# zgbkdlm/fbs

Hardware: AMD Instinct MI355X
Metric: particle-steps/sec (N x T per Gibbs sweep) (higher is better)
Workload: dtype f32; 1 GPU; 2-D Gaussian bridge toy (BASELINE config 2): N=65536 particles, T=500 steps, ts=linspace(0,2), analytic score, gibbs_kernel eb=True ef=False marg_y=False, conditional killing resampling; one step = one Gibbs sweep of a batch of 4 chain(s) (reference driver default nchains=4, vmapped); nparticles=65536, nsteps=500, nchains=4, du=1, dv=1, parallelism=1 GPU(s) x 4 independent chain(s) each, no collective

## Files before the change

### fbs_amd/csrc/fbsmi_lg.hip

```cpp
#include <hip/hip_runtime.h>

#include <array>
#include <cmath>
#include <cstdlib>
#include <map>
#include <mutex>
#include <new>
#include <string>
#include <utility>
#include <vector>

#include "../../include/fbsmi.h"
#include "fbsmi_device.h"
#include "fbsmi_em_path.h"
#include "fbsmi_host.h"

namespace fbsmi {

constexpr int kMaxNbSweep = 1024;
constexpr int kNumProfKernels = 3;

struct LgDev {
    int C;
    int Ctot, c0;
// ... 1183 lines not shown
        }
        __syncthreads();
        t2[0] = waves_combine(L.xch[0][0], L.xch[0][1], L.xch[0][2], L.xch[0][3], s2[0], p2[0]);
        t2[1] = waves_combine(L.xch[1][0], L.xch[1][1], L.xch[1][2], L.xch[1][3], s2[1], p2[1]);
    }
    rootW = t2[0];
    last = d.plus1 ? t2[0] + e.xw : t2[0];
    const float Ji = fmaxf(1.0f - (d.plus1 ? t2[1] + e.xj : t2[1]), 0.0f);
    if (tid) L.topW[g] = make_float2(tree_left_sum(p2[0], tid), e.wf);
    const float tile_ref = tree_fold(Ji, e.refsib);
    float bsib[8];
    {
        const int wb = b_ref >> 6;
#pragma unroll
        for (int lv = 0; lv < 6; ++lv) bsib[lv] = L.bc[lv];
        bsib[6] = L.xch[1][wb ^ 1];
        bsib[7] = (wb & 2) ? L.xch[1][0] + L.xch[1][1] : L.xch[1][2] + L.xch[1][3];
    }
    const float rootJ = ref_extra ? t2[1] : tree_fold(tile_ref, bsib);
    const float lastJ = d.plus1 ? rootJ + (ref_extra ? Ji : e.xj) : rootJ;
    if (tid) {
        const int c = __builtin_ctz(tid);
        const bool hit = !ref_extra && b_ref < tid && b_ref >= tid - (1 << c);
        const float left = hit ? tree_fold(tile_ref, bsib, c) : tree_left_sum(p2[1], tid);
        const float jw = d.plus1 ? jprob_at(e.wf, w_max, d.N) : jprob_pow2(e.wf, w_max, inv_n);
        const float jf = tid * kBlock == i_ref ? Ji : (tid < nb ? jw : 0.0f);
        L.topJ[g] = make_float2(left, jf);
    }
    __syncthreads();
    const float q = lastJ * (1.0f - u3);
    const int top_levels = 31 - __builtin_clz(nb);
    float P = 0.0f, E = rootJ;
    int h = tree_walk_n(L.topJ, kBlock / nb, top_levels, q, P, E);
    const int lo0 = (h - kBlock) * kBlock;
    const float wj = d.w[lo0 + tid];
    float s1[1], t1s[1];
    TreePath p1[1];
    s1[0] = lo0 + tid == i_ref ? Ji : (d.plus1 ? jprob_at(wj, w_max, d.N) : jprob_pow2(wj, w_max, inv_n));
    const float xj = s1[0];
    block_upsweep_n<1>(s1, p1, L.xch[4], t1s);
    if (tid) L.tileJ[g] = make_float2(tree_left_sum(p1[0], tid), xj);
    __syncthreads();
    h = tree_walk_n(L.tileJ, 1, 6, q, P, E);
    {
        const float2 a = L.tileJ[h];
        const float4 c = *reinterpret_cast<const float4*>(L.tileJ + 2 * h);
        const bool g1 = tree_walk(a, q, P, E);
        const float tt = P + (g1 ? c.x : c.z);
        const bool gl = q <= E;
        E = gl ? tt : E;
        h = 4 * h + (g1 ? 0 : 2) + (gl ? 0 : 1);
    }
    const int leaf = lo0 + h - kBlock;
    return q <= E ? leaf : leaf + 1;
}

__device__ __forceinline__ void tree_search_lds(const TreeLds& L, int nb, float q, float& P, float& E, int& tile, int& h) {
    h = tree_walk_n(L.topW, kBlock / nb, 31 - __builtin_clz(nb), q, P, E);
    tile = h - kBlock;
    h = tree_walk_n(L.midW + tile * kMidN, 1, kMidLv, q, P, E);
}

struct TreeRound {
    float s1, y1, s2l, y2l, s2r, y2r, s3a, y3a, s3b, y3b, s3c, y3c, s3d, y3d;
};

__device__ __forceinline__ TreeRound tree_round_load(const LgDev& d, int tile, int h) {
    const float2* tr = d.trW + (size_t)tile * kTreeNodes;
    const float2 n1 = tr[h];
    const float4 n2 = *reinterpret_cast<const float4*>(tr + 2 * h);
    if constexpr (kMidLv == 4) {
        return TreeRound{n1.x, n1.y, n2.x, n2.y, n2.z, n2.w, 0.f, 0.f, 0.f, 0.f, 0.f, 0.f, 0.f, 0.f};
    } else {
        const float4 n3a = *reinterpret_cast<const float4*>(tr + 4 * h);
        const float4 n3b = *reinterpret_cast<const float4*>(tr + 4 * h + 2);
        return TreeRound{n1.x, n1.y, n2.x, n2.y, n2.z, n2.w, n3a.x, n3a.y, n3a.z, n3a.w, n3b.x, n3b.y, n3b.z, n3b.w};
    }
}

__device__ __forceinline__ int tree_round_walk(const TreeRound r, int tile, int h, float q, float& P, float& E) {
    static_assert(kMidLv == 3 || kMidLv == 4, "the round covers the levels between the LDS part and the last four leaves");
    const bool g1 = tree_walk(make_float2(r.s1, r.y1), q, P, E);
    const bool g2 = tree_walk(make_float2(g1 ? r.s2l : r.s2r, g1 ? r.y2l : r.y2r), q, P, E);
    int h4 = 4 * h + (g1 ? 0 : 2) + (g2 ? 0 : 1);
    if constexpr (kMidLv == 3) {
        const float s3 = g1 ? (g2 ? r.s3a : r.s3b) : (g2 ? r.s3c : r.s3d);
        const float y3 = g1 ? (g2 ? r.y3a : r.y3b) : (g2 ? r.y3c : r.y3d);
        h4 = 2 * h4 + (tree_walk(make_float2(s3, y3), q, P, E) ? 0 : 1);
    }
    return tile * kBlock + (h4 - 64) * 4;
}

__device__ __forceinline__ int tree_leaves_walk(float4 w4, int lo, float q, float P, float E) {
    const bool g4 = tree_walk(make_float2(w4.x + w4.y, w4.z), q, P, E);
    const float tt = P + (g4 ? w4.x : w4.z);
    const bool g5 = q <= E;
    const float e1 = g5 ? tt : E;
    const int leaf = lo + (g4 ? 0 : 2) + (g5 ? 0 : 1);
    return q <= e1 ? leaf : leaf + 1;
}

template <int DMAX>
constexpr bool kEarlyRow = DMAX <= 2;

template <int DMAX>
__device__ __forceinline__ int tree_redraw(const LgDev& d, const float* up, int tile, int h, float q, float P, float E,
                                           float (&ucand)[DMAX]) {
    const int N = d.N;
    const TreeRound rd = tree_round_load(d, tile, h);
    const int lo = tree_round_walk(rd, tile, h, q, P, E);
    const float4 w4 = *reinterpret_cast<const float4*>(d.w + lo);
    float4 ug[DMAX];
    float ue[DMAX];
    if (kEarlyRow<DMAX>) {
        const int en = lo + 4 < N ? lo + 4 : N - 1;
#pragma unroll
        for (int r = 0; r < DMAX; ++r) {
            ug[r] = r < d.du ? *reinterpret_cast<const float4*>(up + (size_t)r * N + lo) : make_float4(0.f, 0.f, 0.f, 0.f);
            ue[r] = r < d.du ? up[(size_t)r * N + en] : 0.0f;
        }
    }
    const int red = tree_leaves_walk(w4, lo, q, P, E);
    if (kEarlyRow<DMAX>) {
        const int k = red - lo;
#pragma unroll
        for (int r = 0; r < DMAX; ++r) {
            const float lo2 = (k & 1) ? ug[r].y : ug[r].x, hi2 = (k & 1) ? ug[r].w : ug[r].z;
            ucand[r] = k >= 4 ? ue[r] : ((k & 2) ? hi2 : lo2);
        }
    }
    return red;
}

__device__ __forceinline__ int tree_build_shared(const LgDev& d, const TreeEntry& e, TreeLds& L, bool builder, int i_ref, float u3,
                                                 float w_max, float inv_n, float& last) {
    __shared__ int Jsh;
    __shared__ float lastsh;
    if (builder) {
        float lastb, rootW;
        const int J = tree_build(d, e, L, i_ref, u3, w_max, inv_n, lastb, rootW);
        if (threadIdx.x == 0) {
            Jsh = J;
            lastsh = lastb;
        }
    } else {
#pragma unroll
        for (int k = 0; k < kTreeBuildBarriers; ++k) __syncthreads();
    }
    __syncthreads();
    last = lastsh;
    return Jsh;
}

template <int DMAX, int HALVES>
__global__ void __launch_bounds__(kBlock * HALVES) k_lg_prop1t(LgDev dd, int s) {
    const LgDev d = chain_view(dd, blockIdx.y);
    __shared__ TreeLds L;
    __shared__ float part[2][4 * HALVES];
    const int N = d.N, tid = threadIdx.x & (kBlock - 1), half = threadIdx.x / kBlock;
    int bx = blockIdx.x;
    if (dd.pin) {
        if (blockIdx.x & 7) return;
        bx = blockIdx.x >> 3;
    }
    const int tileb = bx * HALVES + half;
    const int m = tileb * kBlock + tid;
    const bool live = m < N;
    GibbsStep<DMAX> g = gibbs_step_entry<DMAX>(d, s);
    const float w_max = d.scal[1];
    const float inv_n = 1.0f / (float)N;
    TreeEntry te{};
    if (half == 0) te = tree_entry_loads(d);
    gibbs_step_entry_rows<DMAX>(d, s, g);
    float xi[DMAX];
#pragma unroll
    for (int r = 0; r < DMAX; ++r)
        xi[r] = r < d.du ? normal_at(g.t0, g.t1, (uint64_t)N * d.du, (uint64_t)(live ? m : 0) * d.du + r) : 0.0f;
    float last, rootW;
    int J;
    if (HALVES == 1) {
        J = tree_build(d, te, L, g.i_ref, g.u3, w_max, inv_n, last, rootW);
    } else {
        J = tree_build_shared(d, te, L, half == 0, g.i_ref, g.u3, w_max, inv_n, last);
        rootW = last;
    }
    const int src = live ? roll_source(m, roll_shift(g.j_ref, J, N), N) : 0;
    const float ws = d.w[src];
    float u[DMAX];
    load_row<DMAX>(d, g.up, src, u);
    const float u1 = uniform_at(g.a0, g.a1, (uint64_t)N, (uint64_t)src);
    const float u2 = uniform_at(g.b0, g.b1, (uint64_t)N, (uint64_t)src);
    const float q = last * (1.0f - u2);
    float P = 0.0f, E = rootW;
    int tile, h, red = 0;
    tree_search_lds(L, d.nb - d.plus1, q, P, E, tile, h);
    const bool killed = live && u1 * w_max >= ws;
    float ucand[DMAX];
    if (killed) red = tree_redraw<DMAX>(d, g.up, tile, h, q, P, E, ucand);
    gibbs_slot_gather<DMAX, kEarlyRow<DMAX>>(d, g, s, m, src, killed, red, u, ucand, live);
    const float l = gibbs_slot_finish<DMAX>(d, g, s, m, u, xi, live);
    float mx, sx;
    block_lse_partial_tiles(l, part[0], part[1], mx, sx);
    if (tid == 0) {
        d.bmax[tileb] = mx;
        d.bsumexp[tileb] = sx;
    }
}

template <int DMAX>
constexpr bool kPairNoise = DMAX <= 4;

template <int DMAX, int HALVES>
__global__ void __launch_bounds__(kBlock * HALVES) k_lg_prop1tp(LgDev dd, int s) {
    static_assert(HALVES == 2 || HALVES == 4, "two sides of HALVES / 2 tiles");
    constexpr int HP = HALVES / 2, NP = kBlock * HP;
    const LgDev d = chain_view(dd, blockIdx.y);
    __shared__ TreeLds L;
    __shared__ float part[2][4 * HALVES];
    __shared__ float xish[kPairNoise<DMAX> ? DMAX : 1][NP];
    const int N = d.N, tid = threadIdx.x & (kBlock - 1), half = threadIdx.x / kBlock;
    const bool upper = half >= HP;
    const int pr = (int)threadIdx.x - (upper ? NP : 0);
    const int mL = blockIdx.x * NP + pr;
    const int m = upper ? mL + (N >> 1) : mL;
    const int tileb = m / kBlock;
    GibbsStep<DMAX> g = gibbs_step_entry<DMAX>(d, s);
    const float w_max = d.scal[1];
    const float inv_n = 1.0f / (float)N;
    TreeEntry te{};
    if (half == 0) te = tree_entry_loads(d);
    gibbs_step_entry_rows<DMAX>(d, s, g);
    float xi[DMAX] = {};
    if (!kPairNoise<DMAX>) {
#pragma unroll
        for (int r = 0; r < DMAX; ++r)
            if (r < d.du) xi[r] = normal_at(g.t0, g.t1, (uint64_t)N * d.du, (uint64_t)m * d.du + r);
    } else if (upper) {
#pragma unroll
        for (int r = 0; r < DMAX; ++r) {
            if (r < d.du) {
                uint32_t lo_, hi_;
                random_bits_pair(g.t0, g.t1, (uint64_t)N * d.du, (uint64_t)mL * d.du + r, lo_, hi_);
                xish[r][pr] = normal_from_bits(lo_);
                xi[r] = normal_from_bits(hi_);
            }
        }
    }
    float last;
    const int J = tree_build_shared(d, te, L, half == 0, g.i_ref, g.u3, w_max, inv_n, last);
    const int src = roll_source(m, roll_shift(g.j_ref, J, N), N);
    const float ws = d.w[src];
    float u[DMAX];
    load_row<DMAX>(d, g.up, src, u);
    if (kPairNoise<DMAX> && !upper) {
#pragma unroll
        for (int r = 0; r < DMAX; ++r)
            if (r < d.du) xi[r] = xish[r][pr];
    }
    const float u1 = uniform_at(g.a0, g.a1, (uint64_t)N, (uint64_t)src);
    const float u2 = uniform_at(g.b0, g.b1, (uint64_t)N, (uint64_t)src);
    const float q = last * (1.0f - u2);
    float P = 0.0f, E = last;
    int tile, h, red = 0;
    tree_search_lds(L, d.nb, q, P, E, tile, h);
    const bool killed = u1 * w_max >= ws;
    float ucand[DMAX];
    if (killed) red = tree_redraw<DMAX>(d, g.up, tile, h, q, P, E, ucand);
    gibbs_slot_gather<DMAX, kEarlyRow<DMAX>>(d, g, s, m, src, killed, red, u, ucand);
    const float l = gibbs_slot_finish<DMAX>(d, g, s, m, u, xi);
    float mx, sx;
    block_lse_partial_tiles(l, part[0], part[1], mx, sx);
    if (tid == 0) {
        d.bmax[tileb] = mx;
        d.bsumexp[tileb] = sx;
    }
}

__device__ __forceinline__ float halfwave_max(float m) {
    m = fmaxf(m, tree_partner<1>(m));
    m = fmaxf(m, tree_partner<2>(m));
    m = fmaxf(m, tree_partner<4>(m));
    m = fmaxf(m, tree_partner<8>(m));
    m = fmaxf(m, tree_partner<16>(m));
    return m;
}

__device__ __forceinline__ float halfwave_sum(float s) {
    const int lane = threadIdx.x & 63;
#define FBSMI_HALFWAVE_LEVEL(m, M)                      \
    {                                                   \
        const float o_ = tree_partner<M>(s);            \
        s = ((lane >> m) & 1) ? o_ + s : s + o_;        \
    }
    FBSMI_HALFWAVE_LEVEL(0, 1)
    FBSMI_HALFWAVE_LEVEL(1, 2)
    FBSMI_HALFWAVE_LEVEL(2, 4)
    FBSMI_HALFWAVE_LEVEL(3, 8)
    FBSMI_HALFWAVE_LEVEL(4, 16)
#undef FBSMI_HALFWAVE_LEVEL
    return s;
}

template <int DMAX, int HALVES>
__global__ void __launch_bounds__(kBlock * HALVES) k_lg_prop1th(LgDev dd, int s) {
    static_assert(HALVES == 2 || HALVES == 4, "two sides of HALVES / 2 tiles");
    constexpr int HP = HALVES / 2, NP = kBlock * HP;
    const LgDev d = chain_view(dd, blockIdx.y);
    __shared__ TreeLds L;
    __shared__ __attribute__((aligned(16))) float part[2][2][HP][8];
    __shared__ float xish[kPairNoise<DMAX> ? DMAX : 1][2 * NP];
    const int N = d.N, hN = N >> 1, tid = threadIdx.x, lane = threadIdx.x & 63, wv = threadIdx.x >> 6;
    const int hw = lane >> 5;
    const bool builder = tid < kBlock;
    const int pr = wv * 32 + (lane & 31);
    const int mL = blockIdx.x * NP + pr;
    const int m = mL + (hw ? hN : 0);
    const int ts = wv >> 3, bk = wv & 7;
    const int tileb = blockIdx.x * HP + ts + (hw ? d.nb >> 1 : 0);
    GibbsStep<DMAX> g = gibbs_step_entry<DMAX>(d, s);
    const float w_max = d.scal[1];
    const float inv_n = 1.0f / (float)N;
    TreeEntry te{};
    if (builder) te = tree_entry_loads(d);
    gibbs_step_entry_rows<DMAX>(d, s, g);
    float xi[DMAX] = {};
    if (!kPairNoise<DMAX>) {
#pragma unroll
        for (int r = 0; r < DMAX; ++r)
            if (r < d.du) xi[r] = normal_at(g.t0, g.t1, (uint64_t)N * d.du, (uint64_t)m * d.du + r);
    } else if (tid >= NP) {
        const int p = tid - NP, own = (p >> 5) * 64 + (p & 31);
        const int mp = blockIdx.x * NP + p;
#pragma unroll
        for (int r = 0; r < DMAX; ++r) {
            if (r < d.du) {
                uint32_t lo_, hi_;
                random_bits_pair(g.t0, g.t1, (uint64_t)N * d.du, (uint64_t)mp * d.du + r, lo_, hi_);
                xish[r][own] = normal_from_bits(lo_);
                xish[r][own + 32] = normal_from_bits(hi_);
            }
        }
    }
    float last;
    const int J = tree_build_shared(d, te, L, builder, g.i_ref, g.u3, w_max, inv_n, last);
    const int src = roll_source(m, roll_shift(g.j_ref, J, N), N);
    const float ws = d.w[src];
    float u[DMAX];
    load_row<DMAX>(d, g.up, src, u);
    if (kPairNoise<DMAX>) {
#pragma unroll
        for (int r = 0; r < DMAX; ++r)
            if (r < d.du) xi[r] = xish[r][tid];
    }
    const int c = src & (hN - 1);
    const bool swp = (src >= hN) != (hw != 0);
    uint32_t o0, o1;
    threefry2x32(hw ? g.b0 : g.a0, hw ? g.b1 : g.a1, (uint32_t)c, (uint32_t)(c + hN), o0, o1);
    const auto xw = __builtin_amdgcn_permlane32_swap(swp ? o1 : o0, swp ? o0 : o1, false, false);
    const float u1 = fbsmi_bits_to_unit(xw[0]);
    const float u2 = fbsmi_bits_to_unit(xw[1]);
    const float q = last * (1.0f - u2);
    float P = 0.0f, E = last;
    int tile, h, red = 0;
    tree_search_lds(L, d.nb, q, P, E, tile, h);
    const bool killed = u1 * w_max >= ws;
    float ucand[DMAX];
    if (killed) red = tree_redraw<DMAX>(d, g.up, tile, h, q, P, E, ucand);
    gibbs_slot_gather<DMAX, kEarlyRow<DMAX>>(d, g, s, m, src, killed, red, u, ucand);
    const float l = gibbs_slot_finish<DMAX>(d, g, s, m, u, xi);
    float mx, sx;
    {
        const float mw = halfwave_max(l);
        if ((lane & 31) == 0) part[0][hw][ts][bk] = mw;
        __syncthreads();
        const float4 ma = *reinterpret_cast<const float4*>(&part[0][hw][ts][0]);
        const float4 mb = *reinterpret_cast<const float4*>(&part[0][hw][ts][4]);
        mx = fmaxf(fmaxf(fmaxf(ma.x, ma.y), fmaxf(ma.z, ma.w)), fmaxf(fmaxf(mb.x, mb.y), fmaxf(mb.z, mb.w)));
        const float sw_ = halfwave_sum(fbsmi_expf(l - finite_or_zero_f(mx)));
        if ((lane & 31) == 0) part[1][hw][ts][bk] = sw_;
        __syncthreads();
        const float4 sa = *reinterpret_cast<const float4*>(&part[1][hw][ts][0]);
        const float4 sb = *reinterpret_cast<const float4*>(&part[1][hw][ts][4]);
        sx = ((sa.x + sa.y) + (sa.z + sa.w)) + ((sb.x + sb.y) + (sb.z + sb.w));
    }
    if (bk == 0 && (lane & 31) == 0) {
        d.bmax[tileb] = mx;
        d.bsumexp[tileb] = sx;
    }
}

template <int DMAX>
__global__ void __launch_bounds__(kBlock) k_lg_prop2t(LgDev dd, int s) {
    const LgDev d = chain_view(dd, blockIdx.y);
    __shared__ TreeLds L;
    __shared__ float xch2[2][8];
    const int N = d.N, tid = threadIdx.x;
    const int mA = blockIdx.x * kBlock + tid;
    const int m[2] = {mA, mA + (N >> 1)};
    GibbsStep<DMAX> g = gibbs_step_entry<DMAX>(d, s);
    const float w_max = d.scal[1];
    const float inv_n = 1.0f / (float)N;
    const TreeEntry te = tree_entry_loads(d);
    gibbs_step_entry_rows<DMAX>(d, s, g);
    float xi[2][DMAX];
    pair_noise<DMAX>(d, g, mA, xi[0], xi[1]);
    float last;
    float rootW_unused;
    const int J = tree_build(d, te, L, g.i_ref, g.u3, w_max, inv_n, last, rootW_unused);
    int src[2];
    pair_sources(mA, g.j_ref, J, N, src);
    float ws[2], u[2][DMAX];
#pragma unroll
    for (int h2 = 0; h2 < 2; ++h2) {
        ws[h2] = d.w[src[h2]];
#pragma unroll
        for (int r = 0; r < DMAX; ++r) u[h2][r] = r < d.du ? g.up[(size_t)r * N + src[h2]] : 0.0f;
    }
    float u1[2], u2[2];
    pair_uniforms<DMAX>(g, N, src, u1, u2);
    const float qK[2] = {last * (1.0f - u2[0]), last * (1.0f - u2[1])};
    float P[2] = {0.0f, 0.0f}, E[2] = {last, last};
    int tile[2], h[2], hi[2] = {0, 0};
    {
        auto walk2x2 = [&](const float2* hp0, const float2* hp1, int& h0, int& h1) {
            const float2 a0 = hp0[h0], a1 = hp1[h1];
            const float4 c0 = *reinterpret_cast<const float4*>(hp0 + 2 * h0), c1 = *reinterpret_cast<const float4*>(hp1 + 2 * h1);
            const bool g0 = tree_walk(a0, qK[0], P[0], E[0]), g1 = tree_walk(a1, qK[1], P[1], E[1]);
            const bool k0 = tree_walk(g0 ? make_float2(c0.x, c0.y) : make_float2(c0.z, c0.w), qK[0], P[0], E[0]);
            const bool k1 = tree_walk(g1 ? make_float2(c1.x, c1.y) : make_float2(c1.z, c1.w), qK[1], P[1], E[1]);
            h0 = 4 * h0 + (g0 ? 0 : 2) + (k0 ? 0 : 1);
            h1 = 4 * h1 + (g1 ? 0 : 2) + (k1 ? 0 : 1);
        };
        auto walk1x2 = [&](const float2* hp0, const float2* hp1, int& h0, int& h1) {
            const float2 n0 = hp0[h0], n1 = hp1[h1];
            h0 = 2 * h0 + (tree_walk(n0, qK[0], P[0], E[0]) ? 0 : 1);
            h1 = 2 * h1 + (tree_walk(n1, qK[1], P[1], E[1]) ? 0 : 1);
        };
        const int nb = d.nb;
        int h0 = kBlock / nb, h1 = h0, lv = 31 - __builtin_clz(nb);
        for (; lv >= 2; lv -= 2) walk2x2(L.topW, L.topW, h0, h1);
        if (lv) walk1x2(L.topW, L.topW, h0, h1);
        tile[0] = h0 - kBlock;
        tile[1] = h1 - kBlock;
        const float2 *m0 = L.midW + tile[0] * kMidN, *m1 = L.midW + tile[1] * kMidN;
        h0 = h1 = 1;
        static_assert(kMidLv == 3 || kMidLv == 4, "walk of the tile levels kept in LDS");
        walk2x2(m0, m1, h0, h1);
        if (kMidLv == 4) walk2x2(m0, m1, h0, h1);
        else walk1x2(m0, m1, h0, h1);
        h[0] = h0;
        h[1] = h1;
    }
    const bool killed[2] = {u1[0] * w_max >= ws[0], u1[1] * w_max >= ws[1]};
    {
        TreeRound rd0{}, rd1{};
        if (killed[0]) rd0 = tree_round_load(d, tile[0], h[0]);
        if (killed[1]) rd1 = tree_round_load(d, tile[1], h[1]);
        int lo0 = 0, lo1 = 0;
        float4 w40 = make_float4(0.f, 0.f, 0.f, 0.f), w41 = w40;
        if (killed[0]) {
            lo0 = tree_round_walk(rd0, tile[0], h[0], qK[0], P[0], E[0]);
            w40 = *reinterpret_cast<const float4*>(d.w + lo0);
        }
        if (killed[1]) {
            lo1 = tree_round_walk(rd1, tile[1], h[1], qK[1], P[1], E[1]);
            w41 = *reinterpret_cast<const float4*>(d.w + lo1);
        }
        if (killed[0]) hi[0] = tree_leaves_walk(w40, lo0, qK[0], P[0], E[0]);
        if (killed[1]) hi[1] = tree_leaves_walk(w41, lo1, qK[1], P[1], E[1]);
    }
    float lnew[2];
#pragma unroll
    for (int h2 = 0; h2 < 2; ++h2) {
        gibbs_slot_gather<DMAX, false>(d, g, s, m[h2], src[h2], killed[h2], hi[h2], u[h2]);
        lnew[h2] = gibbs_slot_finish<DMAX>(d, g, s, m[h2], u[h2], xi[h2]);
    }
    float mxA, sxA, mxB, sxB;
    block_lse_partial2(lnew[0], lnew[1], xch2[0], xch2[1], mxA, sxA, mxB, sxB);
    if (tid == 0) {
        const int tb = blockIdx.x + (d.nb >> 1);
        d.bmax[blockIdx.x] = mxA;
        d.bsumexp[blockIdx.x] = sxA;
        d.bmax[tb] = mxB;
        d.bsumexp[tb] = sxB;
    }
}

template <int DMAX>
__global__ void __launch_bounds__(kBlock) k_lg_prop2(LgDev dd, int s) {
    const LgDev d = chain_view(dd, blockIdx.y);
    __shared__ float xch[2][8];
    __shared__ __attribute__((aligned(16))) float heapW[kHeapSizeW];
    __shared__ float heapJ[kHeapSizeJ];
    __shared__ float win[kBlock];
    const int N = d.N;
    const int mA = blockIdx.x * kBlock + threadIdx.x;
    const int m[2] = {mA, mA + (N >> 1)};
// ... 1612 lines not shown
                r = f[i] * r + sq[i] * z[i];
                if (live) vs[(size_t)(T - 1 - k0 - i) * dv + j] = r;
            }
        }
    }
    if (live) syT[j] = r;
    __syncthreads();
    for (int u = threadIdx.x; u < p.du; u += blockDim.x) {
        double s = 0.0;
        for (int cc = 0; cc < dv; ++cc) s = s + p.gain[(size_t)u * dv + cc] * ((double)syT[cc] - p.m_v[cc]);
        p.mcond[(size_t)b * p.du + u] = (float)(p.m_u[u] + s);
    }
}

__global__ void __launch_bounds__(kFsBlockMax) k_fs_tail(PmDev p) {
    const int b = blockIdx.y;
    const float* row0 = p.usT + (size_t)b * p.N * p.du;
    for (int r = threadIdx.x; r < p.du; r += blockDim.x) p.uT[(size_t)b * p.du + r] = row0[r];
    if (threadIdx.x == 0) p.log_ell[b] = p.ell[b];
}

struct FsEmDev {
    EmTables t;
    const float *x0_mean, *x0_chol;
    uint32_t* ekeys;
};

constexpr int kFsEmKeysLds = 1024;

template <bool SLAB>
__global__ void __launch_bounds__(kEmPathMaxD) k_fs_front_em(PmDev p, FsEmDev e) {
    __shared__ float xs[2 * kEmPathMaxD];
    __shared__ uint32_t sk[4];
    __shared__ uint32_t skeys[SLAB ? 2 : 2 * kFsEmKeysLds];
    __shared__ float sz[kEmPathMaxD], syT[kEmPathMaxD];
    const int b = blockIdx.y, i = threadIdx.x;
    const int T = p.T, du = p.du, dv = p.dv, D = du + dv;
    if (i == 0) {
        const uint32_t k0 = p.ikeys[2 * b], k1 = p.ikeys[2 * b + 1];
        uint32_t f0, f1, g0, g1;
        split_at(k0, k1, 3, 0, f0, f1);
        split_at(k0, k1, 3, 2, g0, g1);
        p.fkeys[2 * b] = g0;
        p.fkeys[2 * b + 1] = g1;
        split_at(g0, g1, 2, 0, p.pk[4 * b], p.pk[4 * b + 1]);
        split_at(f0, f1, 2, 0, sk[0], sk[1]);
        split_at(f0, f1, 2, 1, sk[2], sk[3]);
    }
    __syncthreads();
    uint32_t* kk = SLAB ? e.ekeys + (size_t)b * T * 2 : skeys;
    for (int k = i; k < T; k += blockDim.x) split_at(sk[2], sk[3], T, k, kk[2 * k], kk[2 * k + 1]);
    const bool proper = e.x0_chol != nullptr;
    float x = 0.0f;
    if (i < du) {
        x = normal_at(sk[0], sk[1], (uint64_t)du, (uint64_t)i);
        sz[i] = x;
    } else if (i < D) {
        x = p.y0[i - du];
    }
    __syncthreads();
    if (proper && i < du) {
        float acc = sz[0] * e.x0_chol[i];
        for (int c = 1; c < du; ++c) acc = acc + sz[c] * e.x0_chol[(size_t)c * du + i];
        x = e.x0_mean[i] + acc;
    }
    float* vs = p.vs + (size_t)b * ((size_t)T + 1) * dv;
    const int col = i - du;
    if (i >= du && i < D) vs[(size_t)T * dv + col] = x;
    const uint64_t n = (uint64_t)e.t.nsub * (uint64_t)D;
    float last = x;
    em_path_run(e.t, T, D, x, xs,
                [&](int k, int j) { return normal_at(kk[2 * k], kk[2 * k + 1], n, (uint64_t)j * D + i); },
                [&](int k, float v) {
                    if (i >= du) vs[(size_t)(T - 1 - k) * dv + col] = v;
                    last = v;
                });
    if (i >= du && i < D) syT[col] = last;
    __syncthreads();
    if (i < du) {
        double s = 0.0;
        for (int cc = 0; cc < dv; ++cc) s = s + p.gain[(size_t)i * dv + cc] * ((double)syT[cc] - p.m_v[cc]);
        p.mcond[(size_t)b * du + i] = (float)(p.m_u[i] + s);
    }
}

}

using namespace fbsmi;

__global__ void k_xcc_probe(int* out) {
    if (threadIdx.x == 0) {
        uint32_t id;
        asm volatile("s_getreg_b32 %0, hwreg(HW_REG_XCC_ID)" : "=s"(id));
        out[blockIdx.x] = (int)(id & 15);
    }
}

static bool xcd_round_robin_holds() {
    static const int ok = [] {
        if (const char* e = getenv("FBSMI_PIN_CHECK"))
            if (atoi(e) == 0) return 1;
        constexpr int kProbeBlocks = 64;
        int* dev = nullptr;
        int host[kProbeBlocks];
        if (hipMalloc(&dev, sizeof(host)) != hipSuccess) return 0;
        bool good = hipMemset(dev, 0xff, sizeof(host)) == hipSuccess;
        if (good) {
            k_xcc_probe<<<kProbeBlocks, 64, 0, nullptr>>>(dev);
            good = hipMemcpy(host, dev, sizeof(host), hipMemcpyDeviceToHost) == hipSuccess;
        }
        (void)hipFree(dev);
        if (!good) return 0;
        unsigned seen = 0;
        for (int b = 0; b < kProbeBlocks; ++b) {
            if (host[b] < 0 || host[b] > 15 || host[b] != host[b & 7]) return 0;
            if (b < 8) seen |= 1u << host[b];
        }
        return __builtin_popcount(seen) == 8 ? 1 : 0;
    }();
    return ok != 0;
}

constexpr int kStreamPool = 4;
static hipStream_t pool_stream(int g) {
    static std::mutex mu;
    static std::map<int, std::array<hipStream_t, kStreamPool>> pools;
    int dev = 0;
    (void)hipGetDevice(&dev);
    const int i = ((g % kStreamPool) + kStreamPool) % kStreamPool;
    std::lock_guard<std::mutex> lock(mu);
    hipStream_t& slot = pools[dev][i];
    if (!slot) {
        hipStream_t st = nullptr;
        if (hipStreamCreateWithFlags(&st, hipStreamNonBlocking) != hipSuccess) return nullptr;
        slot = st;
    }
    return slot;
}

struct fbsmi_lg_sweep {
    LgDev d{};
    int items = 1, dmax = 2;
    std::vector<void*> allocs;
    hipStream_t stream = nullptr;
    hipEvent_t ev_in = nullptr, ev_out = nullptr;
    hipGraphExec_t graph_single = nullptr;
    hipGraphExec_t graph_chain = nullptr;
    bool profile = false;
    int two_slot_prop = -1;
    bool tree_step = true;
    bool tree_plus1 = true;
    int tree_halves = -1;
    bool halfwave = true;
    bool pin = true;
    bool wide_pin = true;
    bool em = false;
    EmDev emd{};
    bool bridge = false;
    BridgeDev brd{};
    std::vector<hipEvent_t> prof_ev[kNumProfKernels];
    double prof_us[kNumProfKernels] = {0, 0, 0};
    int64_t prof_n[kNumProfKernels] = {0, 0, 0};
};

namespace {

void read_switches(fbsmi_lg_sweep* s) {
    auto env = [](const char* name, int unset) {
        const char* e = getenv(name);
        return e ? atoi(e) : unset;
    };
    if (const char* e = getenv("FBSMI_TWO_SLOT_PROP")) s->two_slot_prop = atoi(e) != 0 ? 1 : 0;
    if (const char* e = getenv("FBSMI_TREE_HALVES")) s->tree_halves = atoi(e) == 1 ? 1 : (atoi(e) == 4 ? 4 : 2);
    s->tree_step = env("FBSMI_TREE_STEP", 1) != 0;
    s->tree_plus1 = env("FBSMI_TREE_PLUS1", 1) != 0;
    s->halfwave = env("FBSMI_PROP_HALFWAVE", 1) != 0;
    s->pin = env("FBSMI_PIN", 1) != 0;
    s->wide_pin = env("FBSMI_WIDE_PIN", 1) != 0;
}

template <typename T>
int dev_alloc(fbsmi_lg_sweep* s, T** p, size_t count) {
    void* q = nullptr;
    FBSMI_HIP_TRY(hipMalloc(&q, sizeof(T) * (count ? count : 1)));
    FBSMI_HIP_TRY(hipMemset(q, 0, sizeof(T) * (count ? count : 1)));
    s->allocs.push_back(q);
    *p = (T*)q;
    return 0;
}

struct Slab {
    std::vector<std::pair<void**, size_t>> reqs;
    size_t bytes = 0;

    template <typename T>
    void request(T** p, size_t count) {
        reqs.push_back({(void**)p, bytes});
        bytes += (sizeof(T) * (count ? count : 1) + 255) & ~(size_t)255;
    }

    hipError_t commit(void** base) {
        hipError_t e = hipMalloc(base, bytes ? bytes : 256);
        if (e == hipSuccess) e = hipMemset(*base, 0, bytes ? bytes : 256);
        if (e != hipSuccess) return e;
        for (auto& r : reqs) *r.first = (char*)*base + r.second;
        reqs.clear();
        return hipSuccess;
    }
};

#define LG_DMAX(s, ...)                                                       \
    do {                                                                      \
        if ((s)->dmax == 1) { constexpr int DMAX = 1; __VA_ARGS__; }          \
        else if ((s)->dmax == 2) { constexpr int DMAX = 2; __VA_ARGS__; }     \
        else if ((s)->dmax == 4) { constexpr int DMAX = 4; __VA_ARGS__; }     \
        else { constexpr int DMAX = 16; __VA_ARGS__; }                        \
    } while (0)
#define LG_ITEMS(s, ...)                                                      \
    do {                                                                      \
        if ((s)->items == 1) { constexpr int ITEMS = 1; __VA_ARGS__; }        \
        else if ((s)->items == 4) { constexpr int ITEMS = 4; __VA_ARGS__; }   \
        else { constexpr int ITEMS = 16; __VA_ARGS__; }                       \
    } while (0)

struct ProfScope {
    fbsmi_lg_sweep* s;
    int which;
    hipStream_t st;
    ProfScope(fbsmi_lg_sweep* s_, int which_, hipStream_t st_) : s(s_), which(which_), st(st_) { mark(); }
    ~ProfScope() { mark(); }
    void mark() {
        if (s->profile) {
            hipEvent_t e;
            hipEventCreate(&e);
            hipEventRecord(e, st);
            s->prof_ev[which].push_back(e);
        }
    }
};

int launch_status(const char* what) {
    hipError_t e = hipGetLastError();
    return e == hipSuccess ? FBSMI_OK : fail(FBSMI_ERR_HIP, std::string(what) + " launch: " + hipGetErrorString(e));
}

int grid_1d(int64_t n, int per_block, int cap) {
    const int64_t g = (n + per_block - 1) / per_block;
    return (int)(g < 1 ? 1 : (g > cap ? cap : g));
}

struct WideGeom {
    int nrt, Kp, S;
    size_t lds;
    int nst;
    int u_tiles;
    int v_tile0;
    explicit WideGeom(const LgDev& d)
        : nrt((d.D + kWideTile - 1) / kWideTile), Kp((d.D + 15) / 16 * 16), S(wide_plane_row(Kp)), lds(wide_lds_bytes(S)),
          nst((d.N + kWideTile - 1) / kWideTile), u_tiles((d.du + kWideTile - 1) / kWideTile), v_tile0(d.du / kWideTile) {}
    int v_tiles() const { return nrt - v_tile0; }
};


void sweep_prologue(fbsmi_lg_sweep* s, hipStream_t st, int chain, const WideGeom& w) {
    const LgDev& d = s->d;
    const dim3 gtile(d.nb, d.C);
    k_lg_keys<<<dim3(1, d.C), kBlock, 0, st>>>(d, chain);
    if (s->em) {
        k_lg_em_noise<<<dim3(grid_1d((int64_t)d.T * s->emd.t.nsub * d.D, 256, 1024), d.C), 256, 0, st>>>(d, s->emd);
        k_lg_em_path<<<dim3(1, d.C), (unsigned)((d.D + 63) / 64 * 64), 0, st>>>(d, s->emd, 0);
    } else {
        k_lg_noise<<<dim3(grid_1d((int64_t)d.T * d.D, 256, 1024), d.C), 256, 0, st>>>(d);
        if (s->bridge)
            k_lg_bridge_noise<<<dim3(grid_1d((int64_t)d.T * ((s->brd.nsub * d.dv + 1) / 2), kBlock, 1024), d.C), kBlock, 0, st>>>(d, s->brd);
        k_lg_path<<<dim3((d.D + 63) / 64, d.C), 64, 0, st>>>(d, 0);
        if (s->bridge) k_lg_bridge<<<dim3(1, d.C), (unsigned)((d.dv + 63) / 64 * 64), 0, st>>>(d, s->brd);
    }
    if (d.wide) {
        k_lgw_init<<<gtile, kBlock, 0, st>>>(d);
        if (d.ef) {
            k_lgw_gemm<3><<<dim3(w.nst * w.v_tiles(), d.C), kBlock, w.lds, st>>>(d, 0, w.v_tile0, w.v_tiles(), w.Kp, w.S, 2, 1);
            if (d.N > kBlock) k_lgw_lse<<<gtile, kBlock, 0, st>>>(d);
        }
    } else LG_ITEMS(s, LG_DMAX(s, k_lg_init<ITEMS, DMAX><<<gtile, kBlock, 0, st>>>(d)));
}

void sweep_one_tile_persistent(fbsmi_lg_sweep* s, hipStream_t st) {
    const LgDev& d = s->d;
    LG_DMAX(s, k_lg_sweep1<DMAX><<<dim3(1, d.C), kBlock, 0, st>>>(d));
}

void sweep_one_tile_stepwise(fbsmi_lg_sweep* s, hipStream_t st, const WideGeom& w) {
    const LgDev& d = s->d;
    const int gwide = w.nst * w.nrt;
    const bool pinned = d.wide && s->wide_pin && xcd_round_robin_holds() && d.C == 1 && gwide <= 32;
    const int extra = grid_1d((int64_t)d.N * d.du, 1024, 16);
    for (int k = 0; k < d.T; ++k) {
        ProfScope p(s, 2, st);
        if (pinned) k_lgw_gemm<1><<<dim3(gwide * 8, d.C), kBlock, w.lds, st>>>(d, k, 0, w.nrt, w.Kp, w.S, 3, 8 + ((2 * d.c0) & 7));
        else if (d.wide) k_lgw_gemm<1><<<dim3(gwide + extra, d.C), kBlock, w.lds, st>>>(d, k, 0, w.nrt, w.Kp, w.S, 3, 0);
        else LG_DMAX(s, k_lg_step1<DMAX><<<dim3(1, d.C), kBlock, 0, st>>>(d, k));
    }
}

void step_norm_cdf(fbsmi_lg_sweep* s, hipStream_t st, int k, bool tree, dim3 g, const LgDev& dk) {
    {
        ProfScope p(s, 0, st);
        if (tree) k_lg_norm<1, 0, true><<<dim3(g.x * (dk.pin ? 8 : 1), g.y), kBlock, 0, st>>>(dk, k);
        else LG_ITEMS(s, k_lg_norm<ITEMS, 0><<<g, kBlock, 0, st>>>(dk, k));
    }
    if (tree) return;
    ProfScope p(s, 1, st);
    LG_ITEMS(s, k_lg_cdf<ITEMS, 0><<<g, kBlock, 0, st>>>(dk, k));
}

void sweep_steps_wide(fbsmi_lg_sweep* s, hipStream_t st, const WideGeom& w) {
    const LgDev& d = s->d;
    const dim3 gtile(d.nb, d.C), gwide(w.nst * w.nrt, d.C);
    constexpr int64_t kFatMin = 700;
    const bool fat = (int64_t)gwide.x * d.C > kFatMin;
    const bool fat_rowsum = fat && (d.D & 3) == 0 && (d.du & 3) == 0;
    LgDev dz = d;
    dim3 gz = gtile;
    if (fat) {
        const int64_t third = (((int64_t)d.N * d.du + 1) / 2 + 2) / 3;
        dz.nz = grid_1d(third, kBlock, 1024);
        gz = dim3(gtile.x + dz.nz, gtile.y);
    }
    for (int k = 0; k < d.T; ++k) {
        step_norm_cdf(s, st, k, false, gz, dz);
        ProfScope p(s, 2, st);
        k_lgw_anc<<<gz, kBlock, 0, st>>>(dz, k);
        if (fat_rowsum) k_lgw_gemm_fat<true><<<dim3(w.nst, d.C), kBlock, w.lds, st>>>(d, k, w.nrt, w.Kp, w.S);
        else if (fat) k_lgw_gemm_fat<false><<<dim3(w.nst, d.C), kBlock, w.lds, st>>>(d, k, w.nrt, w.Kp, w.S);
        else k_lgw_gemm<0><<<gwide, kBlock, w.lds, st>>>(d, k, 0, w.nrt, w.Kp, w.S, 3, 0);
        if (fat_rowsum) k_lg_lwpart<<<gtile, kBlock, 0, st>>>(d);
        else k_lgw_lse<<<gtile, kBlock, 0, st>>>(d);
    }
}

void sweep_steps_narrow(fbsmi_lg_sweep* s, hipStream_t st) {
    const LgDev& d = s->d;
    const int nb = d.nb;
    const dim3 gtile(nb, d.C);
    const bool two_slot = s->items == 1 && d.N % (2 * kBlock) == 0 &&
                          (s->two_slot_prop == 1 || (s->two_slot_prop < 0 && (int64_t)nb * d.C >= 5 * 256));
    const bool tree = s->tree_step && d.trW;
    for (int k = 0; k < d.T; ++k) {
        step_norm_cdf(s, st, k, tree, gtile, d);
        ProfScope p(s, 2, st);
        if (tree && two_slot && !d.plus1) {
            LG_DMAX(s, k_lg_prop2t<DMAX><<<dim3(nb / 2, d.C), kBlock, 0, st>>>(d, k));
        } else if (tree && !d.plus1 && nb % 4 == 0 && s->tree_halves == 4) {
            if (s->halfwave) LG_DMAX(s, k_lg_prop1th<DMAX, 4><<<dim3(nb / 4, d.C), 4 * kBlock, 0, st>>>(d, k));
            else LG_DMAX(s, k_lg_prop1tp<DMAX, 4><<<dim3(nb / 4, d.C), 4 * kBlock, 0, st>>>(d, k));
        } else if (tree && !d.plus1 && nb % 2 == 0 && (s->tree_halves == 2 || (s->tree_halves < 0 && (int64_t)nb * d.C >= 2 * 256))) {
            if (s->halfwave) LG_DMAX(s, k_lg_prop1th<DMAX, 2><<<dim3(nb / 2, d.C), 2 * kBlock, 0, st>>>(d, k));
            else LG_DMAX(s, k_lg_prop1tp<DMAX, 2><<<dim3(nb / 2, d.C), 2 * kBlock, 0, st>>>(d, k));
        } else if (tree) {
            LG_DMAX(s, k_lg_prop1t<DMAX, 1><<<dim3(nb * (d.pin ? 8 : 1), d.C), kBlock, 0, st>>>(d, k));
        } else if (two_slot) {
            LG_DMAX(s, k_lg_prop2<DMAX><<<dim3(nb / 2, d.C), kBlock, 0, st>>>(d, k));
        } else if (s->items == 1) {
            LG_DMAX(s, k_lg_prop1<DMAX><<<gtile, kBlock, 0, st>>>(d, k));
        } else {
            k_lg_heaps<<<dim3(kHeapSizeW / kBlock, d.C), kBlock, 0, st>>>(d);
            LG_ITEMS(s, LG_DMAX(s, k_lg_propQ<ITEMS, DMAX><<<gtile, kBlock, 0, st>>>(d, k)));
        }
    }
}

void sweep_epilogue(fbsmi_lg_sweep* s, hipStream_t st, int chain) {
    const LgDev& d = s->d;
    const dim3 gone(1, d.C), gtile(d.nb, d.C);
    if (d.eb) {
        LG_ITEMS(s, k_lg_norm<ITEMS, 1><<<gtile, kBlock, 0, st>>>(d, d.T));
        LG_ITEMS(s, k_lg_cdf<ITEMS, 1><<<gtile, kBlock, 0, st>>>(d, d.T));
        k_lg_force_move<<<gone, 64, 0, st>>>(d);
        const int gpath = (d.D + 63) / 64;
        if (s->em) k_lg_em_path<<<dim3(1, d.C), (unsigned)((d.D + 63) / 64 * 64), 0, st>>>(d, s->emd, 1);
        else k_lg_path<<<dim3(gpath > (d.T + 64) / 64 ? gpath : (d.T + 64) / 64, d.C), 64, 0, st>>>(d, 1);
    } else {
        LG_ITEMS(s, k_lg_norm<ITEMS, 2><<<gtile, kBlock, 0, st>>>(d, d.T));
        LG_ITEMS(s, k_lg_cdf<ITEMS, 2><<<gtile, kBlock, 0, st>>>(d, d.T));
        k_lg_backscan<<<gone, 256, 0, st>>>(d);
    }
    k_lg_export<<<dim3(grid_1d((int64_t)d.N * d.du, 256, 2048), d.C), 256, 0, st>>>(d);
    if (chain) {
        k_lg_advance<<<gone, 256, 0, st>>>(d);
        k_lg_advance_key<<<1, 64, 0, st>>>(d);
    }
}

int enqueue_sweep(fbsmi_lg_sweep* s, hipStream_t st, int chain) {
    const LgDev& d = s->d;
    const WideGeom w(d);
    sweep_prologue(s, st, chain, w);
    if (d.N <= kBlock) {
        if (d.wide || s->profile) sweep_one_tile_stepwise(s, st, w);
        else sweep_one_tile_persistent(s, st);
        if (d.wide) k_lgw_lse<<<dim3(d.nb, d.C), kBlock, 0, st>>>(d);
        else k_lg_lwpart<<<dim3(d.nb, d.C), kBlock, 0, st>>>(d);
    } else if (d.wide) sweep_steps_wide(s, st, w);
    else sweep_steps_narrow(s, st);
    sweep_epilogue(s, st, chain);
    return launch_status("sweep");
}

int run_sweep(fbsmi_lg_sweep* s, int chain, int use_graph) {
    return launch_captured(chain ? s->graph_chain : s->graph_single, s->stream, use_graph && !s->profile,
                           [&] { return enqueue_sweep(s, s->stream, chain); });
}

int join_in(fbsmi_lg_sweep* s, hipStream_t ust) {
    FBSMI_HIP_TRY(hipEventRecord(s->ev_in, ust));
    FBSMI_HIP_TRY(hipStreamWaitEvent(s->stream, s->ev_in, 0));
    return FBSMI_OK;
}

int join_out(fbsmi_lg_sweep* s, hipStream_t ust) {
    FBSMI_HIP_TRY(hipEventRecord(s->ev_out, s->stream));
    FBSMI_HIP_TRY(hipStreamWaitEvent(ust, s->ev_out, 0));
    return FBSMI_OK;
}

int collect_profile(fbsmi_lg_sweep* s) {
    if (!s->profile) return FBSMI_OK;
    FBSMI_HIP_TRY(hipStreamSynchronize(s->stream));
    for (int w = 0; w < kNumProfKernels; ++w) {
        auto& v = s->prof_ev[w];
        for (size_t i = 0; i + 1 < v.size(); i += 2) {
            float ms = 0.f;
            if (hipEventElapsedTime(&ms, v[i], v[i + 1]) == hipSuccess) {
                s->prof_us[w] += (double)ms * 1000.0;
                s->prof_n[w] += 1;
            }
        }
        for (auto e : v) hipEventDestroy(e);
        v.clear();
    }
    return FBSMI_OK;
}

}

extern "C" {

int fbsmi_lg_sweep_create(const fbsmi_lg_model* m, int32_t nparticles, int explicit_backward, int explicit_final,
                          int store_path, int32_t nchains, fbsmi_lg_sweep** out) {
    if (!m || !out || nparticles < 1 || m->du < 1 || m->dv < 1 || m->T < 1 || nchains < 1 || nchains > 65535)
        return fail(FBSMI_ERR_ARG, "lg_sweep_create: bad arguments");
    if (!m->G || !m->g || !m->sd || !m->lognorm || !m->F || !m->sqQ)
        return fail(FBSMI_ERR_ARG, "lg_sweep_create: null model table");
    const int D = m->du + m->dv;
    const bool wide = m->du > 16 || m->dv > 16;
    if (wide && (m->du > 128 || m->dv > 128))
        return fail(FBSMI_ERR_UNSUPPORTED, "lg_sweep: du, dv > 128 are not supported by the fused sweep");

    if (wide && (explicit_final ? nparticles + 1 : nparticles) > 131072)
        return fail(FBSMI_ERR_UNSUPPORTED, "lg_sweep: du, dv > 16 with more than 131072 particles is not supported");
    if (!explicit_backward && !store_path)
        return fail(FBSMI_ERR_ARG, "lg_sweep_create: explicit_backward=0 needs store_path (As, uss)");
    fbsmi_lg_sweep* s = new (std::nothrow) fbsmi_lg_sweep();
    if (!s) return fail(FBSMI_ERR_ARG, "out of host memory");
    auto bail = [s](int code, const std::string& msg) {
        fbsmi_lg_sweep_destroy(s);
        return fail(code, msg);
    };
    LgDev& d = s->d;
    d.C = nchains;
    d.Ctot = nchains;
    d.c0 = 0;
    d.nparticles = nparticles;
    d.N = explicit_final ? nparticles + 1 : nparticles;
    d.du = m->du;
    d.dv = m->dv;
    d.D = D;
    d.T = m->T;
    d.eb = explicit_backward ? 1 : 0;
    d.ef = explicit_final ? 1 : 0;
    d.store = store_path ? 1 : 0;
    d.dt = m->dt;
    d.lw_init = (float)(-log((double)nparticles));
    d.G = m->G; d.g = m->g; d.sd = m->sd; d.lognorm = m->lognorm; d.F = m->F; d.sqQ = m->sqQ;
    d.levels = bisect_levels(d.N);
    d.wide = wide ? 1 : 0;
    read_switches(s);
    s->items = fbsmi_tile_items(d.N);
    const int maxd = m->du > m->dv ? m->du : m->dv;
    s->dmax = maxd <= 1 ? 1 : (maxd <= 2 ? 2 : (maxd <= 4 ? 4 : 16));
    const int tile = kBlock * s->items;
    d.nb = (d.N + tile - 1) / tile;
    if (d.nb > kMaxNbSweep) return bail(FBSMI_ERR_UNSUPPORTED, "lg_sweep: more than 4M particles per device not supported yet");
    if (store_path) {
        const double bytes = (((double)d.T * d.N * 4.0) + ((double)(d.T + 1) * d.N * (d.du + 1) * 4.0)) * nchains;
        if (bytes > 200e9) return bail(FBSMI_ERR_UNSUPPORTED, "lg_sweep: path storage (T,N,du) does not fit device memory");
    }
    const size_t N = d.N, T = d.T, C = nchains;
    Slab slab;
    slab.request(&d.key, 2);
    slab.request(&d.keys, 2 * C);
    slab.request(&d.x0, C * d.du);
    slab.request(&d.y0, d.dv);
    slab.request(&d.bs, C * (T + 1));
    slab.request(&d.keytab, C * 8 * T);
    slab.request(&d.misc, C * 16);
    slab.request(&d.xi1, C * T * D);
    slab.request(&d.xi2, C * T * D);
    slab.request(&d.path, 1);
    slab.request(&d.us_star, C * (T + 1) * d.du);
// ... 753 lines not shown
```

Measured before the change: 19.36 billion particle-steps/s.

## Split per-step tree build across wave roles with wave-level J search

Adds a ROLES variant of the halfwave propagation kernel, on by default via FBSMI_J_WAVE. The shared tree build is split across waves: wave 0 computes the conditional-killing index J with a register and readlane tree walk, wave 1 builds the weight-side top tree into LDS, and waves 2-3 stage the mid-level tree from global memory. The aim is to cut the serial per-block tree-build latency and its barrier chain before the propagation work starts. In exchange the code grows more complex, relies on nb fitting in 256 tiles, and adds a wave-uniform search path that must match the old sampling exactly.

Measured after the change: 21.19 billion particle-steps/s (median of 6 runs). +9.4%, better.

```diff
diff --git a/fbs_amd/csrc/fbsmi_lg.hip b/fbs_amd/csrc/fbsmi_lg.hip
--- a/fbs_amd/csrc/fbsmi_lg.hip
+++ b/fbs_amd/csrc/fbsmi_lg.hip
@@ -1359,6 +1359,183 @@
     return Jsh;
 }
 
+struct WaveTree {
+    float x[4];
+    float s01, s23;
+    TreePath p;
+};
+
+__device__ __forceinline__ float wave_tree_upsweep(WaveTree& t) {
+    t.s01 = t.x[0] + t.x[1];
+    t.s23 = t.x[2] + t.x[3];
+    return wave_upsweep(t.s01 + t.s23, t.p);
+}
+
+__device__ __forceinline__ float lane_read(float v, int l) {
+    return __builtin_bit_cast(float, __builtin_amdgcn_readlane(__builtin_bit_cast(int, v), l));
+}
+__device__ __forceinline__ int wave_uniform(int v) { return __builtin_amdgcn_readfirstlane(v); }
+
+__device__ __forceinline__ float wave_tree_left_sum(const TreePath p, int lane) {
+    float v = p.ls[5];
+    v = (lane & 16) ? p.ls[4] : v;
+    v = (lane & 8) ? p.ls[3] : v;
+    v = (lane & 4) ? p.ls[2] : v;
+    v = (lane & 2) ? p.ls[1] : v;
+    v = (lane & 1) ? p.ls[0] : v;
+    return v;
+}
+
+template <int C>
+__device__ __forceinline__ float wave_tree_half(const WaveTree& t, int lo) {
+    const int ml = (lo + (1 << C)) >> 2;
+    if constexpr (C >= 2) return lane_read(t.p.ls[C - 2], ml);
+    else if constexpr (C == 1) return lane_read(t.s01, ml);
+    else return (lo & 2) ? lane_read(t.x[2], ml) : lane_read(t.x[0], ml);
+}
+template <int C>
+__device__ __forceinline__ float wave_tree_mid(const float (&y)[4], int lo) {
+    const int ml = (lo + (1 << C)) >> 2;
+    if constexpr (C >= 2) return lane_read(y[0], ml);
+    else if constexpr (C == 1) return lane_read(y[2], ml);
+    else return (lo & 2) ? lane_read(y[3], ml) : lane_read(y[1], ml);
+}
+
+__device__ __forceinline__ float4 tile_values4(const float* p, int nb, int lane) {
+    const int t = 4 * lane;
+    if (nb >= 4) return t < nb ? *reinterpret_cast<const float4*>(p + t) : make_float4(0.f, 0.f, 0.f, 0.f);
+    return make_float4(t < nb ? p[t] : 0.0f, t + 1 < nb ? p[t + 1] : 0.0f, 0.f, 0.f);
+}
+
+struct RoleEntry {
+    float4 sj, wf;
+    float refsib[8];
+};
+
+__device__ __forceinline__ float4 role_entry_loads(const LgDev& d, int i_ref, RoleEntry& e) {
+    const int tid = threadIdx.x, nb = d.nb;
+    float4 wref = make_float4(0.f, 0.f, 0.f, 0.f);
+    if (tid < 64) {
+        e.sj = tile_values4(d.bsumJ, nb, tid);
+        e.wf = tile_values4(d.wfirst, nb, tid);
+        wref = *reinterpret_cast<const float4*>(d.w + i_ref / kBlock * kBlock + 4 * tid);
+#pragma unroll
+        for (int lv = 0; lv < 8; ++lv) e.refsib[lv] = d.scal[4 + lv];
+    }
+    return wref;
+}
+
+__device__ __forceinline__ float wave_tree_w_side(float4 sw, float4 wf, TreeLds& L) {
+    const int lane = threadIdx.x & 63;
+    WaveTree t;
+    t.x[0] = sw.x; t.x[1] = sw.y; t.x[2] = sw.z; t.x[3] = sw.w;
+    const float total = wave_tree_upsweep(t);
+    const int t0 = 4 * lane;
+    if (lane) L.topW[tree_mid_node(t0)] = make_float2(wave_tree_left_sum(t.p, lane), wf.x);
+    L.topW[tree_mid_node(t0 + 1)] = make_float2(t.x[0], wf.y);
+    L.topW[tree_mid_node(t0 + 2)] = make_float2(t.s01, wf.z);
+    L.topW[tree_mid_node(t0 + 3)] = make_float2(t.x[2], wf.w);
+    return total;
+}
+
+__device__ __forceinline__ int wave_tree_J(const LgDev& d, const RoleEntry& e, const float4 wref, int i_ref, float u3, float w_max,
+                                           float inv_n) {
+    const int lane = threadIdx.x & 63, nb = d.nb;
+    i_ref = wave_uniform(i_ref);
+    const int b_ref = i_ref / kBlock, lb = b_ref >> 2;
+    WaveTree t;
+    t.x[0] = e.sj.x; t.x[1] = e.sj.y; t.x[2] = e.sj.z; t.x[3] = e.sj.w;
+    const float wf[4] = {e.wf.x, e.wf.y, e.wf.z, e.wf.w};
+    float jq[4];
+#pragma unroll
+    for (int i = 0; i < 4; ++i) jq[i] = jprob_pow2(wf[i], w_max, inv_n);
+    const float total = wave_tree_upsweep(t);
+    const float Ji = fmaxf(1.0f - total, 0.0f);
+    float jf[4];
+#pragma unroll
+    for (int i = 0; i < 4; ++i) jf[i] = (4 * lane + i) * kBlock == i_ref ? Ji : (4 * lane + i < nb ? jq[i] : 0.0f);
+    const float tile_ref = tree_fold(Ji, e.refsib);
+    float bsib[8];
+    {
+        const int pos = b_ref & 3;
+        const float s0 = (pos & 2) ? ((pos & 1) ? t.x[2] : t.x[3]) : ((pos & 1) ? t.x[0] : t.x[1]);
+        bsib[0] = lane_read(s0, lb);
+        bsib[1] = lane_read((pos & 2) ? t.s01 : t.s23, lb);
+        bsib[2] = lane_read(t.p.ls[0], lb); bsib[3] = lane_read(t.p.ls[1], lb); bsib[4] = lane_read(t.p.ls[2], lb);
+        bsib[5] = lane_read(t.p.ls[3], lb); bsib[6] = lane_read(t.p.ls[4], lb); bsib[7] = lane_read(t.p.ls[5], lb);
+    }
+    const float rootJ = tree_fold(tile_ref, bsib);
+    const float q = rootJ * (1.0f - u3);
+    const int top_levels = 31 - __builtin_clz(nb);
+    float P = 0.0f, E = rootJ;
+    int lo = 0;
+#define FBSMI_JTOP_LEVEL(C)                                                                 \
+    if (C < top_levels) {                                                                   \
+        const int mid = lo + (1 << C);                                                      \
+        float left = wave_tree_half<C>(t, lo);                                              \
+        if (b_ref >= lo && b_ref < mid) left = tree_fold(tile_ref, bsib, C);                \
+        lo = wave_uniform(tree_walk(make_float2(left, wave_tree_mid<C>(jf, lo)), q, P, E) ? lo : mid); \
+    }
+    FBSMI_JTOP_LEVEL(7) FBSMI_JTOP_LEVEL(6) FBSMI_JTOP_LEVEL(5) FBSMI_JTOP_LEVEL(4)
+    FBSMI_JTOP_LEVEL(3) FBSMI_JTOP_LEVEL(2) FBSMI_JTOP_LEVEL(1) FBSMI_JTOP_LEVEL(0)
+#undef FBSMI_JTOP_LEVEL
+    const int lo0 = lo * kBlock;
+    float w0 = wref.x, w1 = wref.y, w2 = wref.z, w3 = wref.w;
+    if (lo != b_ref) {
+        const float4 w4 = *reinterpret_cast<const float4*>(d.w + lo0 + 4 * lane);
+        w0 = w4.x; w1 = w4.y; w2 = w4.z; w3 = w4.w;
+    }
+    const int m0 = lo0 + 4 * lane;
+    t.x[0] = m0 == i_ref ? Ji : jprob_pow2(w0, w_max, inv_n);
+    t.x[1] = m0 + 1 == i_ref ? Ji : jprob_pow2(w1, w_max, inv_n);
+    t.x[2] = m0 + 2 == i_ref ? Ji : jprob_pow2(w2, w_max, inv_n);
+    t.x[3] = m0 + 3 == i_ref ? Ji : jprob_pow2(w3, w_max, inv_n);
+    wave_tree_upsweep(t);
+    lo = 0;
+#define FBSMI_JTILE_LEVEL(C) \
+    lo = wave_uniform(tree_walk(make_float2(wave_tree_half<C>(t, lo), wave_tree_mid<C>(t.x, lo)), q, P, E) ? lo : lo + (1 << C));
+    FBSMI_JTILE_LEVEL(7) FBSMI_JTILE_LEVEL(6) FBSMI_JTILE_LEVEL(5) FBSMI_JTILE_LEVEL(4) FBSMI_JTILE_LEVEL(3) FBSMI_JTILE_LEVEL(2)
+#undef FBSMI_JTILE_LEVEL
+    const int ml = lo >> 2;
+    const float x0 = lane_read(t.x[0], ml), x2 = lane_read(t.x[2], ml), s01 = lane_read(t.s01, ml);
+    const bool g1 = tree_walk(make_float2(s01, x2), q, P, E);
+    const float tt = P + (g1 ? x0 : x2);
+    const bool gl = q <= E;
+    E = gl ? tt : E;
+    const int leaf = lo0 + lo + (g1 ? 0 : 2) + (gl ? 0 : 1);
+    return q <= E ? leaf : leaf + 1;
+}
+
+__device__ __forceinline__ int tree_build_roles(const LgDev& d, const RoleEntry& e, const float4 wref, TreeLds& L, int i_ref, float u3,
+                                                float w_max, float inv_n, float& last) {
+    __shared__ int Jsh;
+    __shared__ float lastsh;
+    const int tid = threadIdx.x, lane = tid & 63, wv = tid >> 6, nb = d.nb;
+    if (wv == 0) {
+        const int J = wave_tree_J(d, e, wref, i_ref, u3, w_max, inv_n);
+        if (lane == 0) Jsh = J;
+    } else if (wv == 1) {
+        const float total = wave_tree_w_side(tile_values4(d.bsumw, nb, lane), tile_values4(d.wfirst, nb, lane), L);
+        if (lane == 0) lastsh = total;
+    } else if (wv < 4) {
+        constexpr int STN = 2 * 64, STK = kMidN / 2 * kBlock / STN;
+        float4 stg[STK];
+#pragma unroll
+        for (int k = 0; k < STK; ++k) {
+            const int idx = tid - 2 * 64 + STN * k;
+            stg[k] = idx < kMidN / 2 * nb ? reinterpret_cast<const float4*>(d.trWtop)[idx] : make_float4(0.f, 0.f, 0.f, 0.f);
+        }
+#pragma unroll
+        for (int k = 0; k < STK; ++k) {
+            const int idx = tid - 2 * 64 + STN * k;
+            if (idx < kMidN / 2 * nb) reinterpret_cast<float4*>(L.midW)[idx] = stg[k];
+        }
+    }
+    __syncthreads();
+    last = lastsh;
+    return Jsh;
+}
+
 template <int DMAX, int HALVES>
 __global__ void __launch_bounds__(kBlock * HALVES) k_lg_prop1t(LgDev dd, int s) {
     const LgDev d = chain_view(dd, blockIdx.y);
@@ -1508,7 +1685,7 @@
     return s;
 }
 
-template <int DMAX, int HALVES>
+template <int DMAX, int HALVES, bool ROLES>
 __global__ void __launch_bounds__(kBlock * HALVES) k_lg_prop1th(LgDev dd, int s) {
     static_assert(HALVES == 2 || HALVES == 4, "two sides of HALVES / 2 tiles");
     constexpr int HP = HALVES / 2, NP = kBlock * HP;
@@ -1528,7 +1705,10 @@
     const float w_max = d.scal[1];
     const float inv_n = 1.0f / (float)N;
     TreeEntry te{};
-    if (builder) te = tree_entry_loads(d);
+    RoleEntry re;
+    float4 wref = make_float4(0.f, 0.f, 0.f, 0.f);
+    if (ROLES) wref = role_entry_loads(d, g.i_ref, re);
+    else if (builder) te = tree_entry_loads(d);
     gibbs_step_entry_rows<DMAX>(d, s, g);
     float xi[DMAX] = {};
     if (!kPairNoise<DMAX>) {
@@ -1549,7 +1729,8 @@
         }
     }
     float last;
-    const int J = tree_build_shared(d, te, L, builder, g.i_ref, g.u3, w_max, inv_n, last);
+    const int J = ROLES ? tree_build_roles(d, re, wref, L, g.i_ref, g.u3, w_max, inv_n, last)
+                        : tree_build_shared(d, te, L, builder, g.i_ref, g.u3, w_max, inv_n, last);
     const int src = roll_source(m, roll_shift(g.j_ref, J, N), N);
     const float ws = d.w[src];
     float u[DMAX];
@@ -3468,6 +3649,7 @@
     bool tree_plus1 = true;
     int tree_halves = -1;
     bool halfwave = true;
+    bool j_wave = true;
     bool pin = true;
     bool wide_pin = true;
     bool em = false;
@@ -3491,6 +3673,7 @@
     s->tree_step = env("FBSMI_TREE_STEP", 1) != 0;
     s->tree_plus1 = env("FBSMI_TREE_PLUS1", 1) != 0;
     s->halfwave = env("FBSMI_PROP_HALFWAVE", 1) != 0;
+    s->j_wave = env("FBSMI_J_WAVE", 1) != 0;
     s->pin = env("FBSMI_PIN", 1) != 0;
     s->wide_pin = env("FBSMI_WIDE_PIN", 1) != 0;
 }
@@ -3531,6 +3714,11 @@
         else if ((s)->dmax == 2) { constexpr int DMAX = 2; __VA_ARGS__; }     \
         else if ((s)->dmax == 4) { constexpr int DMAX = 4; __VA_ARGS__; }     \
         else { constexpr int DMAX = 16; __VA_ARGS__; }                        \
+    } while (0)
+#define LG_ROLES(s, ...)                                                      \
+    do {                                                                      \
+        if ((s)->j_wave) { constexpr bool ROLES = true; __VA_ARGS__; }        \
+        else { constexpr bool ROLES = false; __VA_ARGS__; }                   \
     } while (0)
 #define LG_ITEMS(s, ...)                                                      \
     do {                                                                      \
@@ -3668,10 +3856,10 @@
         if (tree && two_slot && !d.plus1) {
             LG_DMAX(s, k_lg_prop2t<DMAX><<<dim3(nb / 2, d.C), kBlock, 0, st>>>(d, k));
         } else if (tree && !d.plus1 && nb % 4 == 0 && s->tree_halves == 4) {
-            if (s->halfwave) LG_DMAX(s, k_lg_prop1th<DMAX, 4><<<dim3(nb / 4, d.C), 4 * kBlock, 0, st>>>(d, k));
+            if (s->halfwave) LG_ROLES(s, LG_DMAX(s, k_lg_prop1th<DMAX, 4, ROLES><<<dim3(nb / 4, d.C), 4 * kBlock, 0, st>>>(d, k)));
             else LG_DMAX(s, k_lg_prop1tp<DMAX, 4><<<dim3(nb / 4, d.C), 4 * kBlock, 0, st>>>(d, k));
         } else if (tree && !d.plus1 && nb % 2 == 0 && (s->tree_halves == 2 || (s->tree_halves < 0 && (int64_t)nb * d.C >= 2 * 256))) {
-            if (s->halfwave) LG_DMAX(s, k_lg_prop1th<DMAX, 2><<<dim3(nb / 2, d.C), 2 * kBlock, 0, st>>>(d, k));
+            if (s->halfwave) LG_ROLES(s, LG_DMAX(s, k_lg_prop1th<DMAX, 2, ROLES><<<dim3(nb / 2, d.C), 2 * kBlock, 0, st>>>(d, k)));
             else LG_DMAX(s, k_lg_prop1tp<DMAX, 2><<<dim3(nb / 2, d.C), 2 * kBlock, 0, st>>>(d, k));
         } else if (tree) {
             LG_DMAX(s, k_lg_prop1t<DMAX, 1><<<dim3(nb * (d.pin ? 8 : 1), d.C), kBlock, 0, st>>>(d, k));
```
